# eggersn/DistributedFFT

Measured on AMD Instinct MI355X. Metric: 3D FFT GFLOP/s (5N^3 log2 N^3 per direction), forward+inverse, higher is better.
Workload: dtype f64

## Files before the change

### distributedfft_amd/__init__.py

```python
from ._lib import DfftError, LIB_PATH
from .api import (All2All, Comm, Configurations, DeviceBuffer, FORWARD, GlobalSize, INVERSE, MPI_Type, MPIcuFFT,
                  MPIcuFFT_Pencil, MPIcuFFT_Pencil_Opt1, MPIcuFFT_Slab, MPIcuFFT_Slab_Opt1, MPIcuFFT_Slab_Y_Then_ZX, MPIcuFFT_Slab_Z_Then_YX,
                  MPIcuFFT_Slab_Z_Then_YX_Opt1, Partition, Partition_Dimensions,
                  Peer2Peer, Pencil_Partition, SPECTRAL_OP, Slab_Partition, Streams, Sync, axis_plan_info, fft1d_batched, kernel_info, last_placement_info)
```

### distributedfft_amd/_lib.py

```python
import ctypes as C
import os

_HERE = os.path.dirname(os.path.abspath(__file__))
LIB_PATH = os.environ.get("DFFT_AMD_LIBRARY") or os.path.join(_HERE, "libdfft_amd.so")

ALLTOALLV_FN = C.CFUNCTYPE(C.c_int, C.c_void_p, C.c_void_p, C.POINTER(C.c_size_t), C.POINTER(C.c_size_t),
                           C.c_void_p, C.POINTER(C.c_size_t), C.POINTER(C.c_size_t), C.POINTER(C.c_int),
                           C.c_int, C.c_int, C.c_void_p)
SENDRECV_LIST_FN = C.CFUNCTYPE(C.c_int, C.c_void_p, C.c_int, C.POINTER(C.c_int), C.POINTER(C.c_void_p), C.POINTER(C.c_size_t),
                               C.c_int, C.POINTER(C.c_int), C.POINTER(C.c_void_p), C.POINTER(C.c_size_t), C.c_void_p)


class Config(C.Structure):
    _fields_ = [("cuda_aware", C.c_int), ("warmup_rounds", C.c_int), ("comm_method", C.c_int),
                ("send_method", C.c_int), ("comm_method2", C.c_int), ("send_method2", C.c_int)]


class PassDesc(C.Structure):
    _fields_ = [("na", C.c_uint32), ("LB", C.c_uint32), ("nb", C.c_uint32), ("LA", C.c_uint32), ("T2shift", C.c_uint32),
                ("load_kind", C.c_int32), ("store_kind", C.c_int32), ("swap", C.c_int32), ("shift", C.c_int32),
                ("KS_in", C.c_uint64), ("KS_out", C.c_uint64), ("AS_in", C.c_uint64), ("AS_out", C.c_uint64),
                ("IA", C.c_uint64), ("IB", C.c_uint64), ("SK", C.c_uint64), ("SB", C.c_uint64),
                ("a_fastest", C.c_int32), ("xcd_swizzle", C.c_int32),
                ("in_off", C.c_uint64), ("out_off", C.c_uint64),
# ... 67 lines not shown
    ("dfft_enable_phase_timing", _i, [_vp, _i]),
    ("dfft_fft1d_batched", _i, [_i, _sz, _sz, _vp, _vp, _i, _vp]),
    ("dfft_fft1d_batched_ex", _i, [_i, _sz, _sz, _vp, _vp, _i, _vp, _i, _i]),
    ("dfft_get_pass_choices", _i, [_vp, C.POINTER(_i), C.POINTER(_i), C.POINTER(_i)]),
    ("dfft_debug_get_pass", _i, [_vp, C.c_char_p, _i, C.POINTER(PassDesc)]),
    ("dfft_debug_get_chain", _i, [_vp, _i, _i, C.POINTER(ChainStep), _i, C.POINTER(_i)]),
    ("dfft_debug_trace_chain", _i, [_vp, _i, _i, C.POINTER(TraceOp), _i, C.POINTER(_i)]),
    ("dfft_debug_get_point_table", _i, [_vp, C.c_char_p, _i, _i, C.POINTER(C.c_uint64), C.POINTER(C.c_uint32),
                                        C.POINTER(C.c_uint32), _sz, _psz]),
    ("dfft_last_error", C.c_char_p, []),
    ("dfft_version", C.c_char_p, []),
    ("dfft_kernel_info", _i, [_i, _sz, C.POINTER(_i), C.POINTER(_i), C.POINTER(_i), C.POINTER(_i)]),
    ("dfft_axis_plan_info", _i, [_i, _sz, _i, C.POINTER(_sz)]),
    ("dfft_malloc", _i, [_sz, _sz, C.POINTER(_vp)]),
    ("dfft_free", _i, [_vp]),
    ("dfft_last_placement_info", _i, [C.c_char_p, _sz]),
    ("dfft_tune_variants", _i, [_vp, _vp, _vp, _vp, C.POINTER(C.c_float), _i, C.POINTER(_i)]),
    ("dfft_tune_placement", _i, [_vp, _vp, _i, C.POINTER(_vp), C.POINTER(_vp), C.POINTER(C.c_float), _i, C.POINTER(_i)]),
]

_lib = None


def lib():
    global _lib
    if _lib is None:
        if not os.path.exists(LIB_PATH):
            raise ImportError(
                f"{LIB_PATH} is missing: build it with `python -c 'import __graft_entry__ as g; g.build()'` "
                "or `make -C distributedfft_amd/csrc` (hipcc, gfx950).  There is no CPU fallback.")
# ... 17 lines not shown
```

### distributedfft_amd/api.py

```python
import ctypes as C
from dataclasses import dataclass

from . import _lib
from ._lib import Config, DfftError, check, lib

Peer2Peer, All2All = 0, 1
Sync, Streams, MPI_Type = 0, 1, 2
FORWARD, INVERSE = -1, 1
SPECTRAL_OP = 2


class GlobalSize:

    def __init__(self, Nx, Ny, Nz):
        self.Nx, self.Ny, self.Nz = int(Nx), int(Ny), int(Nz)
        self.Nz_out = self.Nz // 2 + 1


class Partition:

    def __init__(self, P1=1, P2=1):
        self.P1, self.P2 = int(P1), int(P2)


# ... 83 lines not shown
            lib().dfft_free(C.c_void_p(self.address))
        self.address = 0

    def __del__(self):
        try:
            self.free()
        except Exception:
            pass


def last_placement_info():
    import json
    buf = C.create_string_buffer(1024)
    check(lib().dfft_last_placement_info(buf, 1024))
    return json.loads(buf.value.decode())


class Comm:

    def __init__(self, handle, nranks, rank=None, keep=None):
        self._h, self.nranks, self.rank, self._keep = handle, nranks, rank, keep

    @classmethod
    def local(cls, nranks):
        h = C.c_void_p()
        check(lib().dfft_comm_create_local(nranks, C.byref(h)))
        return cls(h, nranks)

    @classmethod
    def rccl(cls, unique_id, nranks, rank):
# ... 365 lines not shown
```

### distributedfft_amd/csrc/alloc.hip

```cpp
#include <hip/hip_runtime.h>
#include <stdint.h>
#include <stdio.h>
#include <stdlib.h>

#include <algorithm>
#include <atomic>
#include <chrono>
#include <map>
#include <mutex>
#include <string>
#include <vector>

#include "alloc.hpp"
#include "host_common.hpp"

namespace dfft {

struct DevAlloc { size_t bytes, chunk; int device; };
static std::mutex g_alloc_mu;
static std::map<void *, DevAlloc> g_allocs;

static std::atomic<uintptr_t> g_next_va{0};
static hipError_t reserve_fresh(void **va, size_t total, size_t align)
{
// ... 24 lines not shown
        std::lock_guard<std::mutex> lk(g_alloc_mu);
        auto it = g_allocs.find(ptr);
        if (it != g_allocs.end()) { rec = it->second; g_allocs.erase(it); }
    }
    if (!rec.chunk) { HIP_TRY(hipFree(ptr)); return 0; }
    int cur = -1;
    (void)hipGetDevice(&cur);
    const bool hop = rec.device >= 0 && cur >= 0 && rec.device != cur;
    if (hop) HIP_TRY(hipSetDevice(rec.device));
    hipError_t e = hipDeviceSynchronize();
    for (size_t off = 0; off < rec.bytes && e == hipSuccess; off += rec.chunk) e = hipMemUnmap(static_cast<char *>(ptr) + off, rec.chunk);
    if (e == hipSuccess) e = hipMemAddressFree(ptr, rec.bytes);
    if (hop) (void)hipSetDevice(cur);
    if (e != hipSuccess) { set_error(std::string("dfft_free: ") + hipGetErrorString(e)); return (int)e; }
    return 0;
}
struct AllocTimes { double create = 0, map = 0, release = 0; };
static thread_local AllocTimes g_alloc_times;
static double seconds_since(std::chrono::steady_clock::time_point t0) { return std::chrono::duration<double>(std::chrono::steady_clock::now() - t0).count(); }

int dev_alloc(size_t bytes, size_t chunk_mib, void **out, int spread)
{
    *out = nullptr;
    g_alloc_times = AllocTimes();
    if (!bytes) return fail(ERR_ARG, "zero-sized allocation");
    if (!chunk_mib) {
        int dev0 = -1;
        (void)hipGetDevice(&dev0);
        HIP_TRY(hipMalloc(out, bytes));
        std::lock_guard<std::mutex> lk(g_alloc_mu);
// ... 276 lines not shown
```

### distributedfft_amd/csrc/alloc.hpp

```cpp
#pragma once
#include <stddef.h>

namespace dfft {
int dev_alloc(size_t bytes, size_t chunk_mib, void **out, int spread = 1);
int dev_alloc_default(size_t bytes, void **out);
int dev_free(void *ptr);
size_t default_chunk_mib();
int placement_info_json(char *buf, size_t capacity);
}
```

### distributedfft_amd/csrc/dfft.hip

```cpp
#include "../../include/dfft_c.h"
#include "comm.hpp"
#include "dfft_internal.hpp"
#include "fft_pass.hip.h"

#include <math.h>
#include <stdlib.h>
#include <string.h>
#include <algorithm>
#include <atomic>
#include <chrono>
#include <complex>
#include <functional>
#include <map>
#include <mutex>
#include <string>
#include <vector>

#include "alloc.hpp"
#include "host_common.hpp"
#include "plan.hpp"

namespace dfft {

static thread_local std::string g_error;
// ... 266 lines not shown
        PassArgs A = P;
        natural_side(A, false);
        layout(A, true, qout);
        PassArgs L3 = A;
        L3.lb = 0; L3.real_mode = 0; L3.swap = 0; L3.shift = 0;
        natural_side(L3, true);
        L3.out = nullptr;
        TRY(level(L3, 1, true));
        PassArgs L4 = A;
        L4.lb = 6; L4.lbL = (uint32_t)ax.N; L4.lbK = (uint32_t)NK; L4.lbtab = ax.chirp; L4.real_mode = real_mode;
        TRY(level(L4, 2, qout));
    }
    return 0;
}

static int launch(dfft_plan *p, const Launch &L, int form, int axis, bool conj, const char *in, char *out, hipStream_t stream)
{
    if (L.args.ntiles == 0) return 0;
    const Axis &ax = p->ax[axis];
    PassArgs A = L.args;
    A.in = in + L.in_off; A.out = out + L.out_off; A.tw = ax.tw; A.debug = p->opt.debug;
    if (conj) A.swap = 1;
    fill_tables(p, L, A);
    const int real_mode = form == FORM_REAL_Z1 || form == FORM_REAL_LINES ? 1 : form == FORM_REAL_Z2 ? 2 : 0;
    const size_t NK = real_mode ? ax.N / 2 + 1 : ax.N;
    if (real_mode && (form == FORM_REAL_LINES ? p->yreal_native : p->zreal_native)) {
        A.tw2 = p->tw_zr;
        const bool z = form != FORM_REAL_LINES;
        const int M = (int)((z ? p->Nz : p->Ny) / 2), variant = z ? p->opt.real_variant : 0;
        const int r = p->prec == DFFT_F64 ? launch_real_f64(M, real_mode, variant, A, stream) : launch_real_f32(M, real_mode, variant, A, stream);
        if (r != 0) return fail(r == -1 ? ERR_UNSUPPORTED : r, "real pass launch failed for length " + std::to_string(2 * M));
        return 0;
    }
    if (!ax.bluestein) {
        if (real_mode) return fail(ERR_UNSUPPORTED, "real pass without a packed or Bluestein plan");
        return launch_pass(p->prec, (int)ax.N, form == FORM_FWD ? p->vfwd[axis] : form == FORM_INV ? p->vinv[axis] : 0, A, stream);
// ... 87 lines not shown
    if (C < 2) return 1;
    return want < 0 ? (C >= 3 ? 2 : 1) : (want > 1 ? 2 : 1);
}

static hipEvent_t pipe_event(dfft_plan *p, size_t i)
{
    Pipeline &pl = p->pl;
    while (pl.ev.size() <= i) {
        hipEvent_t e = nullptr;
        if (hipEventCreateWithFlags(&e, hipEventDisableTiming) != hipSuccess) return nullptr;
        pl.ev.push_back(e);
    }
    return pl.ev[i];
}

static const Chain &chain_of(const dfft_plan *p, int direction, int dims)
{
    const Pipeline &pl = p->pl;
    if (direction == DFFT_SPECTRAL_OP) return pl.spec;
    const bool fwd = direction != DFFT_INVERSE;
    if (dims == 3 && one_rank_alternative(p) && !(fwd ? pl.one_fwd : pl.one_inv).steps.empty()) return fwd ? pl.one_fwd : pl.one_inv;
    return fwd ? pl.fwd[dims - 1] : pl.inv[dims - 1];
}

std::vector<Launch> *pass_launches(dfft_plan *p, int k)
{
    static const int alt[6] = {G_SZ, G_SY, G_SX, -1, -1, -1};
    const int g = p->pl.single && one_rank_alternative(p) ? alt[k] : k;
    return g < 0 ? nullptr : &p->pl.groups[g].L;
}

static bool graph_replay(const dfft_plan *p) { return p->opt.graph && p->nranks == 1 && !p->timing && (p->stream || !p->stream_user); }

static bool through_level_scratch(const dfft_plan *p, int form, int axis)
{
// ... 38 lines not shown
    int xchg(int step, int chunk, int s, int ) { ops.push_back(trace_exchange(st, step, chunk, s)); return 0; }
    int record(int s, int e) { ops.push_back(trace_sync(2, s, e)); return 0; }
    int wait(int e, int s) { ops.push_back(trace_sync(3, s, e)); return 0; }
    int begin(int, int) { return 0; }
    int end(int) { return 0; }
};

struct HipSink {
    dfft_plan *p;
    const std::vector<Step> &st;
    int direction;
    void *out;
    const void *in;
    std::vector<dfft_trace_op> *log;
    hipStream_t S[4];
    int open(const StreamUse &use)
    {
        Pipeline &pl = p->pl;
        if (use.compute2 && !pl.compute_stream2) HIP_TRY(hipStreamCreateWithFlags(&pl.compute_stream2, hipStreamNonBlocking));
        if (use.comm && !pl.comm_stream) HIP_TRY(hipStreamCreateWithFlags(&pl.comm_stream, hipStreamNonBlocking));
        if (use.comm2 && !pl.comm_stream2) HIP_TRY(hipStreamCreateWithFlags(&pl.comm_stream2, hipStreamNonBlocking));
        S[S_MAIN] = p->stream; S[S_COMPUTE2] = pl.compute_stream2; S[S_COMM] = pl.comm_stream; S[S_COMM2] = pl.comm_stream2;
        return 0;
    }
    char *buf(int b) const
    {
        return b == BUF_IN ? const_cast<char *>(static_cast<const char *>(in)) : b == BUF_OUT ? static_cast<char *>(out)
                                                                               : static_cast<char *>(p->work_d) + (size_t)b * p->domainsize;
    }
    int kernel(int step, int chunk, int k, int s)
    {
        const Step &t = st[(size_t)step];
        const Group &g = p->pl.groups[t.group];
        if (log) log->push_back(trace_launch(p, st, step, chunk, k, s));
        if (t.group == G_XX) return launch_spectral(p, g.L[(size_t)k], buf(t.src), buf(t.dst), S[s]);
        return launch(p, g.L[(size_t)k], t.form, g.axis, t.conj, buf(t.src), buf(t.dst), S[s]);
    }
    int xchg(int step, int chunk, int s, int ready)
    {
        const Step &t = st[(size_t)step];
        const Pipeline &pl = p->pl;
        const int dir = t.tables ? t.tables : direction;
        const std::vector<A2A> &T = dir == DFFT_INVERSE ? (t.xchg == 1 ? pl.i1 : pl.i2) : (t.xchg == 1 ? pl.f1 : pl.f2);
        if (log) log->push_back(trace_exchange(st, step, chunk, s));
        return exchange_tables(p, t.xchg, T[(size_t)chunk], true, buf(t.dst), buf(st[(size_t)step + 1].src), S[s], s == S_COMM2 ? 1 : 0, 0,
                               pl.ev[(size_t)ready]);
    }
    int record(int s, int e)
    {
        hipEvent_t ev = pipe_event(p, (size_t)e);
        if (!ev) return fail(1, "hipEventCreate failed");
// ... 62 lines not shown
                TRY(sk.xchg((int)s1 - 1, c, Sx, ready));
                if (t.phase >= 0) TRY(sk.end(Sx));
                TRY(record(Sx, xdone[c]));
            }
        }
        xprev = st[s1 - 1].xchg; xn = nchunk;
        if (s1 == st.size() && spread) TRY(join(Sc2, Sc));
    }
    return 0;
}

static int trace_slot(int direction) { return direction == DFFT_SPECTRAL_OP ? 2 : direction == DFFT_INVERSE ? 1 : 0; }

static int run_chain(dfft_plan *p, int direction, int dims, void *out, const void *in)
{
    const Chain &ch = chain_of(p, direction, dims);
    if (ch.steps.empty())
        return direction == DFFT_SPECTRAL_OP ? fail(ERR_STATE, "plan was initialised without option spectral_op")
                                             : fail(ERR_UNSUPPORTED, "the Y_Then_ZX sequence is forward only (as in the reference)");
    const StreamUse use = streams_of(p, ch);
    p->nspans = 0; p->last_dir = direction == DFFT_INVERSE ? DFFT_INVERSE : DFFT_FORWARD;
    std::vector<dfft_trace_op> *log = nullptr;
    if (p->opt.trace) { log = &p->trace_log[trace_slot(direction)]; log->clear(); }
    HipSink sk{p, ch.steps, direction, out, in, log, {}};
    TRY(sk.open(use));
    return schedule_chain(p, ch, use, sk);
}

void graphs_clear(dfft_plan *p)
{
    for (auto &g : p->graphs) if (g.exec) (void)hipGraphExecDestroy(g.exec);
    p->graphs.clear();
}
template <typename F> static int run_graphed(dfft_plan *p, int kind, const void *in, void *out, F &&enqueue)
{
    if (!graph_replay(p) || !p->stream) return enqueue();
    dfft_plan::GraphEntry *e = nullptr;
    for (auto &g : p->graphs) if (g.kind == kind && g.in == in && g.out == out) { e = &g; break; }
    if (e && e->exec) { HIP_TRY(hipGraphLaunch(e->exec, p->stream)); return 0; }
// ... 177 lines not shown
    if (k == "mirror_inverse") return &o.mirror;
    if (k == "point_tables") return &o.tables;
    if (k == "uniform_tables") return &o.uniform_tables;
    if (k == "shift") return &o.shift;
    if (k == "debug_skip") return &o.debug;
    if (k == "real_variant") return &o.real_variant;
    if (k == "single_order") return &o.single_order;
    if (k == "single_layout") return &o.single_layout;
    if (k == "single_pad") return &o.single_pad;
    if (k == "native_mixed") return &o.native_mixed;
    if (k == "graph") return &o.graph;
    if (k == "spectral_layout") return &o.spectral;
    if (k == "spectral_op") return &o.spectral_op;
    if (k == "compute_streams") return &o.compute_streams;
    if (k == "trace") return &o.trace;
    for (int i = 0; i < 6; i++) {
        if (k == std::string("variant_") + kPassNames[i]) return &o.variant[i];
        if (k == std::string("order_") + kPassNames[i]) return &o.order[i];
    }
    return nullptr;
}
int dfft_set_option(dfft_plan *p, const char *key, long value)
{
    if (!p || !key) return fail(ERR_ARG, "null plan or key");
    int *slot = option_slot(p->opt, key);
    if (!slot) return fail(ERR_ARG, std::string("unknown option ") + key);
    if (std::string(key).rfind("variant_", 0) == 0 && (value < -1 || value > 15)) return fail(ERR_ARG, "variant_* must be -1 (the plan's choice) or 0..15");
    *slot = (int)value;
    graphs_clear(p);
    return 0;
}
long dfft_get_option(dfft_plan *p, const char *key)
{
    if (!p || !key) return -1;
    int *slot = option_slot(p->opt, key);
    return slot ? *slot : -1;
}

int dfft_plan_destroy(dfft_plan *p)
{
    if (!p) return 0;
    graphs_clear(p);
    if (p->work_owned && p->work_d) (void)dev_free(p->work_d);
    relay_cache_free(p->relay);
    for (auto &a : p->ax) axis_free(a);
    for (void *t : {p->tw_zr, p->tables_d}) if (t) (void)hipFree(t);
    for (auto &t : p->spans) { if (t.a) (void)hipEventDestroy(t.a); if (t.b) (void)hipEventDestroy(t.b); }
    for (auto &e : p->pl.ev) if (e) (void)hipEventDestroy(e);
    if (p->pl.comm_stream) (void)hipStreamDestroy(p->pl.comm_stream);
    if (p->pl.comm_stream2) (void)hipStreamDestroy(p->pl.comm_stream2);
    if (p->pl.compute_stream2) (void)hipStreamDestroy(p->pl.compute_stream2);
    if (p->stream_owned && p->stream) (void)hipStreamDestroy(p->stream);
    delete p;
    return 0;
}

int dfft_init(dfft_plan *p, size_t Nx, size_t Ny, size_t Nz, int P1, int P2, int c2c, int allocate)
{
    if (!p) return fail(ERR_ARG, "null plan");
    p->initialized = false;
    graphs_clear(p);
    relay_cache_free(p->relay);
    p->relay = nullptr;
    if (!Nx || !Ny || !Nz) return fail(ERR_ARG, "GlobalSize not initialized!");
    if (P1 < 1 || P2 < 1 || P1 * P2 != p->nranks) return fail(ERR_ARG, "Invalid Input Partition!");
    const bool zyx_kind = p->kind == DFFT_SLAB_Z_THEN_YX || p->kind == DFFT_SLAB_Z_THEN_YX_OPT1;
    const bool yzx = p->kind == DFFT_SLAB_Y_THEN_ZX;
    if ((p->kind == DFFT_SLAB || p->kind == DFFT_SLAB_OPT1 || zyx_kind || yzx) && P2 != 1)
        return fail(ERR_ARG, "slab decomposition needs P2 == 1");
    const bool zyx = zyx_kind && P1 > 1;
    if (P1 > MAXSEG || P2 > MAXSEG) return fail(ERR_UNSUPPORTED, "more than 32 ranks per exchange group");
    if ((size_t)P1 > Nx || (!zyx && (size_t)P1 > Ny) || (size_t)P2 > Ny) return fail(ERR_ARG, "partition larger than the grid");
    {
        Axis az, ay, axx;
        const bool mixed = p->opt.native_mixed != 0;
        const int tl = p->opt.two_level;
        const bool zr_native = !yzx && !c2c && tl != 1 && Nz >= 4 && Nz <= 4096 && Nz % 2 == 0 && (is_pow2(Nz) || mixed) &&
                               (p->prec == DFFT_F64 ? real_supported_f64((int)(Nz / 2)) : real_supported_f32((int)(Nz / 2)));
// ... 95 lines not shown
            for (const Launch &L : g.L) {
                const Axis &a = p->ax[g.axis];
                if (a.two) lvb = std::max(lvb, two_level_bytes(L.args, p->TL, a.N, p->esz));
                if (a.longb) lvb = std::max(lvb, long_bytes(L.args, p->TL, a.M, p->esz));
            }
        p->worksize_d = (p->worksize_d + 255) & ~(size_t)255;
        p->lv_off = p->worksize_d;
        p->lv_bytes = (lvb + 255) & ~(size_t)255;
        p->worksize_d += p->lv_bytes;
    }
    {
        PassInfo vi;
        auto has64 = [&](const Axis &a, int role) { return !a.bluestein && pass_info_f64((int)a.N, role, &vi); };
        auto has32 = [&](const Axis &a, int role) { return !a.bluestein && pass_info_f32((int)a.N, role, &vi); };
        for (int k = 0; k < 3; k++) p->vfwd[k] = p->vinv[k] = ROLE_DEFAULT;
        if (p->prec == DFFT_F64) {
            const size_t zs_local = p->zs.empty() ? p->Nzc : p->zs[p->zyx ? (size_t)p->rank % p->zs.size() : (size_t)p->pj % p->zs.size()];
            if (has64(p->ax[2], ROLE_STRIDED_READ) && zs_local % (size_t)p->TL == 0) p->vinv[2] = ROLE_STRIDED_READ;
            if (p->vinv[2] == ROLE_STRIDED_READ && p->P1 == 1 && has64(p->ax[2], ROLE_STRIDED_READ_FUSED)) p->vinv[2] = ROLE_STRIDED_READ_FUSED;
            const int zrole = has64(p->ax[0], ROLE_LINES) ? ROLE_LINES : has64(p->ax[0], ROLE_STREAM) ? ROLE_STREAM : ROLE_DEFAULT;
            if (p->c2c) p->vfwd[0] = p->vinv[0] = zrole;
            if (has64(p->ax[1], ROLE_STREAM)) p->vinv[1] = ROLE_STREAM;
            if (p->opt.spectral) {
                const int xrole = has64(p->ax[2], ROLE_LINES) ? ROLE_LINES : has64(p->ax[2], ROLE_STREAM) ? ROLE_STREAM : ROLE_DEFAULT;
                p->vfwd[2] = p->vinv[2] = xrole;
            }
        } else {
            if (p->c2c && has32(p->ax[0], ROLE_NATURAL_LOAD)) p->vfwd[0] = ROLE_NATURAL_LOAD;
            if (p->c2c && has32(p->ax[0], ROLE_NATURAL_STORE)) p->vinv[0] = ROLE_NATURAL_STORE;
            for (int ax = 1; ax <= 2; ax++)
                if (has32(p->ax[ax], ROLE_TILED)) p->vfwd[ax] = p->vinv[ax] = ROLE_TILED;
            if (has32(p->ax[1], ROLE_TRANSPOSED_STORE)) p->vinv[1] = ROLE_TRANSPOSED_STORE;
            if (p->nranks > 1 && p->ax[1].N >= 2048 && has32(p->ax[1], ROLE_TILED_STREAM)) p->vfwd[1] = ROLE_TILED_STREAM;
            if (p->nranks > 1 && p->ax[2].N >= 2048 && has32(p->ax[2], ROLE_TILED_STREAM)) p->vinv[2] = ROLE_TILED_STREAM;
            if (p->opt.spectral) {
                if (has32(p->ax[2], ROLE_NATURAL_STORE)) p->vfwd[2] = ROLE_NATURAL_STORE;
                if (has32(p->ax[2], ROLE_NATURAL_LOAD_TILED_STORE)) p->vinv[2] = ROLE_NATURAL_LOAD_TILED_STORE;
            }
        }
    }
// ... 88 lines not shown
    }
    for (const Chain *ch : {&chain_of(p, DFFT_FORWARD, 3), &chain_of(p, DFFT_INVERSE, 3), &chain_of(p, DFFT_SPECTRAL_OP, 3)}) {
        HipSink sk{p, ch->steps, DFFT_FORWARD, nullptr, nullptr, nullptr, {}};
        TRY(sk.open(streams_of(p, *ch)));
    }
    return 0;
}

int dfft_set_work_area(dfft_plan *p, void *device, void *host)
{
    (void)host;
    if (!p) return fail(ERR_ARG, "null plan");
    if (!p->initialized) return fail(ERR_STATE, "cannot set work area: plan not initialised");
    graphs_clear(p);
    if (p->work_owned && p->work_d) { (void)dev_free(p->work_d); p->work_d = nullptr; p->work_owned = false; }
    TRY(ensure_device_state(p));
    if (device) {
        p->work_d = device;
    } else {
        TRY(dev_alloc_default(p->worksize_d, &p->work_d));
        p->work_owned = true;
    }
    return 0;
}

int dfft_set_pipeline_chunks(dfft_plan *p, int chunks)
{
    if (!p) return fail(ERR_ARG, "null plan");
    if (chunks < 0) return fail(ERR_ARG, "chunks must be >= 0");
    p->opt.chunks = chunks;
    return 0;
}
int dfft_get_pipeline_chunks(const dfft_plan *p) { return p ? p->pl.C : 0; }

int dfft_set_stream(dfft_plan *p, void *hip_stream)
{
    if (!p) return fail(ERR_ARG, "null plan");
// ... 195 lines not shown
    const Launch *L = find_launch(p, name, index);
    if (!L) return fail(ERR_ARG, "the plan has no such launch");
    const PassArgs &A = L->args;
    memset(d, 0, sizeof(*d));
    d->na = A.na; d->LB = A.LB; d->nb = A.nb; d->LA = A.LA; d->T2shift = A.T2shift;
    d->load_kind = A.load_kind; d->store_kind = A.store_kind; d->swap = A.swap; d->shift = A.shift;
    d->KS_in = A.KS_in; d->KS_out = A.KS_out; d->AS_in = A.AS_in; d->AS_out = A.AS_out;
    d->IA = A.IA; d->IB = A.IB; d->SK = A.SK; d->SB = A.SB; d->a_fastest = A.a_fastest; d->xcd_swizzle = A.xcd_swizzle;
    d->in_off = L->in_off; d->out_off = L->out_off;
    d->lnseg = L->lseg.nseg; d->snseg = L->sseg.nseg;
    for (int s = 0; s < L->lseg.nseg; s++) { d->lstart[s] = L->lseg.start[s]; d->llen[s] = L->lseg.len[s]; d->lbase[s] = L->lseg.base[s]; }
    for (int s = 0; s < L->sseg.nseg; s++) { d->sstart[s] = L->sseg.start[s]; d->slen[s] = L->sseg.len[s]; d->sbase[s] = L->sseg.base[s]; }
    return 0;
}

int dfft_debug_get_chain(const dfft_plan *p, int direction, int dims, dfft_chain_step *steps, int capacity, int *count)
{
    if (!p || !p->initialized) return fail(ERR_STATE, "plan not initialised");
    const bool spec = direction == DFFT_SPECTRAL_OP && dims == 3;
    if (dims < 1 || dims > 3 || (direction != DFFT_FORWARD && direction != DFFT_INVERSE && !spec)) return fail(ERR_ARG, "bad direction or dims");
    const Chain &ch = chain_of(p, direction, dims);
    const std::vector<Step> &st = ch.steps;
    if (count) *count = (int)st.size();
    for (size_t i = 0; i < st.size() && (int)i < capacity; i++) {
        const Step &s = st[i];
        const Group &g = p->pl.groups[s.group];
        dfft_chain_step &d = steps[i];
        memset(&d, 0, sizeof(d));
        strncpy(d.group, g.name, sizeof(d.group) - 1);
        d.axis = g.axis; d.launches = (int32_t)g.L.size(); d.per_chunk = s.per_chunk;
        d.src = s.src; d.dst = s.dst; d.conj = s.conj; d.form = s.form; d.exchange = s.xchg; d.split = ch.split;
        d.tables = s.tables ? s.tables : (direction == DFFT_INVERSE ? DFFT_INVERSE : DFFT_FORWARD);
    }
    return 0;
}

int dfft_debug_trace_chain(const dfft_plan *p, int direction, int dims, dfft_trace_op *ops, int capacity, int *count)
{
    if (!p || !p->initialized) return fail(ERR_STATE, "plan not initialised");
    const bool spec = direction == DFFT_SPECTRAL_OP && (dims == 3 || dims == 0);
    if (dims < 0 || dims > 3 || (direction != DFFT_FORWARD && direction != DFFT_INVERSE && !spec)) return fail(ERR_ARG, "bad direction or dims");
    std::vector<dfft_trace_op> dry;
    if (dims > 0) {
        const Chain &ch = chain_of(p, direction, dims);
        DrySink sk{p, ch.steps, dry};
        TRY(schedule_chain(p, ch, streams_of(p, ch), sk));
    }
    const std::vector<dfft_trace_op> &v = dims > 0 ? dry : p->trace_log[trace_slot(direction)];
    if (count) *count = (int)v.size();
    for (size_t i = 0; i < v.size() && (int)i < capacity; i++) ops[i] = v[i];
    return 0;
}

int dfft_get_pass_choices(const dfft_plan *p, int variant[6], int order[6], int addr64[6])
{
    if (!p || !p->initialized) return fail(ERR_STATE, "plan not initialised");
    for (int k = 0; k < 6; k++) {
        const std::vector<Launch> *v = pass_launches(const_cast<dfft_plan *>(p), k);
        const Launch *L = v && !v->empty() ? &(*v)[0] : nullptr;
// ... 142 lines not shown
    for (int k = 0; k < 8; k++) info[k] = 0;
    info[0] = a.longb ? 3 : a.two ? 2 : a.bluestein ? 1 : 0;
    info[1] = a.M;
    if (a.longb) a = Axis(a.lv[0]);
    for (size_t k = 0; k < a.lv.size(); k++) { info[2 + 3 * k] = a.lv[k].N; info[3 + 3 * k] = a.lv[k].M; info[4 + 3 * k] = a.lv[k].bluestein; }
    return 0;
}

int dfft_malloc(size_t bytes, size_t chunk_mib, void **ptr)
{
    if (!ptr) return fail(ERR_ARG, "null pointer");
    if (chunk_mib == DFFT_CHUNK_DEFAULT) return dev_alloc_default(bytes, ptr);
    return dev_alloc(bytes, chunk_mib, ptr);
}
int dfft_free(void *ptr) { return dev_free(ptr); }
int dfft_last_placement_info(char *buf, size_t capacity)
{
    if (!buf || !capacity) return fail(ERR_ARG, "null buffer");
    return placement_info_json(buf, capacity);
}

}
```

### distributedfft_amd/csrc/pipeline.hip

```cpp
#include <string.h>

#include <algorithm>

#include "host_common.hpp"
#include "plan.hpp"

using namespace dfft;

static PassArgs pass_args(int TL, size_t na, size_t LB, int load_kind, int store_kind, int swap)
{
    PassArgs A;
    memset(&A, 0, sizeof(A));
    A.na = (uint32_t)na; A.LB = (uint32_t)LB; A.nb = (uint32_t)((LB + TL - 1) / TL); A.ntiles = A.na * A.nb;
    A.load_kind = load_kind; A.store_kind = store_kind; A.swap = swap; A.T2shift = ilog2(TL);
    return A;
}

static void set_shift(const dfft_plan *p, PassArgs &X)
{
    const uint32_t TL = (uint32_t)p->TL;
    if (p->opt.shift == 0) return;
    if (p->ax[2].bluestein) return;
    if (p->prec != DFFT_F64 && p->opt.shift != 2) return;
    if (X.AS_out % TL == 0 || X.KS_out % TL != 0 || X.LB < TL) return;
    X.shift = 1;
    X.nb += 1;
    X.ntiles = X.na * X.nb;
}

static std::vector<Launch> &group(Pipeline &pl, int g, size_t n)
{
    pl.groups[g].L.assign(n, Launch());
    return pl.groups[g].L;
}

static void clear(Pipeline &pl)
{
    for (auto &g : pl.groups) g.L.clear();
    for (Chain *c : {&pl.fwd[0], &pl.fwd[1], &pl.fwd[2], &pl.inv[0], &pl.inv[1], &pl.inv[2], &pl.one_fwd, &pl.one_inv, &pl.spec}) *c = Chain();
    pl.single = false;
}

static void seg_push(SegTable &t, size_t start, size_t len, size_t base_elems)
{
    int s = t.nseg++;
    t.start[s] = (uint32_t)start;
    t.len[s] = (uint32_t)len;
    t.base[s] = base_elems;
}

int build_pipeline(dfft_plan *p, Pipeline &pl)
{
    const int TL = p->TL, P1 = p->P1, P2 = p->P2, C = pl.C;
    const size_t xs = p->xs[p->pi], ys = p->ys[p->pj], zs = p->zs[p->pj], yo = p->yo[p->pi];
// ... 183 lines not shown
        const int isrc = P1 > 1 ? (P2 > 1 ? 1 : E) : xd, idst = P2 > 1 ? E : (P1 > 1 ? 1 : 0), zsrc = P2 > 1 ? (P1 > 1 ? 0 : 1) : idst;
        pl.spec.steps = {{G_FZ, zf, BUF_IN, E, -1, x1, false, 1, false, DFFT_FORWARD},
                         {G_FY, FORM_FWD, ysrc, ydst, -1, x2, false, 1, false, DFFT_FORWARD},
                         {G_XX, FORM_FIXED, xsrc, xd, -1, x2, true, 1, false, DFFT_INVERSE},
                         {G_IY, FORM_INV, isrc, idst, -1, x1, true, 1, false, DFFT_INVERSE},
                         {G_IZ, zi, zsrc, BUF_OUT, -1, 0, P2 == 1, 1, false, DFFT_INVERSE}};
        pl.spec.split = true;
    }
    pl.fwd[0].steps = {{G_PZ1, zf, BUF_IN, BUF_OUT}};
    pl.inv[0].steps = {{G_QZ1, zi, BUF_IN, BUF_OUT}};
    pl.fwd[1].steps = {{G_FZ, zf, BUF_IN, 0, -1, x1}, {G_PY2, FORM_FWD, x1, BUF_OUT, -1, 0, P2 == 1}};
    pl.inv[1].steps = {{G_QY2, FORM_INV, BUF_IN, 0, -1, x1}, {G_IZ, zi, x1, BUF_OUT, -1, 0, P2 == 1}};
    if (p->nranks == 1 && p->c2c)
        pl.one_inv.steps = {{G_FZ, FORM_FWD, BUF_IN, 0, 4, 0, false, 1, true}, {G_FY, FORM_FWD, 0, BUF_IN, 2, 0, true, 1, true},
                            {G_FX, FORM_FWD, BUF_IN, BUF_OUT, 0, 0, true, 1, true}};
    return 0;
}

int build_pipeline_zyx(dfft_plan *p, Pipeline &pl)
{
    const int TL = p->TL, P = p->P1, C = pl.C, r = p->pi;
    const size_t xs = p->xs[r], zs = p->zs[r];
    const size_t Ny = p->Ny, Nzc = p->Nzc, e = p->esz;
    const size_t zline_bytes = p->c2c ? p->Nz * e : p->Nz * (e / 2);
    auto base = [&](size_t na, size_t LB, int lk, int sk, int swap) { return pass_args(TL, na, LB, lk, sk, swap); };
    std::vector<size_t> xl, x0;
    split(xs, C, xl, x0);
    std::vector<std::vector<size_t>> xlq(P), x0q(P);
    for (int q = 0; q < P; q++) split(p->xs[q], C, xlq[q], x0q[q]);
    std::vector<std::vector<size_t>> blk(C, std::vector<size_t>(P, 0));
// ... 192 lines not shown
```

### distributedfft_amd/csrc/plan.hpp

```cpp
#pragma once
#include <hip/hip_runtime.h>
#include <stddef.h>
#include <stdint.h>

#include <string>
#include <vector>

#include "../../include/dfft_c.h"
#include "comm.hpp"
#include "dfft_internal.hpp"
#include "fft_pass.hip.h"

namespace dfft {

inline void split(size_t n, int p, std::vector<size_t> &size, std::vector<size_t> &start)
{
    size.assign(p, n / p);
    start.assign(p, 0);
    for (size_t i = 0; i < n % p; i++) size[i]++;
    size_t off = 0;
    for (int i = 0; i < p; i++) { start[i] = off; off += size[i]; }
}

inline bool is_pow2(size_t n) { return n && !(n & (n - 1)); }
// ... 61 lines not shown
    bool whole = false;
    int per_chunk = 1;
    bool conj = false;
    int tables = 0;
};
struct Chain {
    std::vector<Step> steps;
    bool split = false;
};

struct Pipeline {
    int C = 1;
    Group groups[NGROUPS] = {{"fz", 0}, {"fy", 1}, {"fx", 2}, {"ix", 2}, {"iy", 1}, {"iz", 0}, {"pz1", 0}, {"qz1", 0}, {"py2", 1},
                             {"qy2", 1}, {"zy", 1}, {"ziy", 1}, {"zix", 2}, {"yz", 0}, {"sz", 0}, {"sx", 2}, {"sy", 1}, {"xx", 2}};
    Chain fwd[3], inv[3], one_fwd, one_inv;
    Chain spec;
    bool single = false;
    size_t single_work_elems = 0;
    std::vector<A2A> f1, f2, i2, i1;
    std::vector<hipEvent_t> ev;
    hipStream_t comm_stream = nullptr;
    hipStream_t comm_stream2 = nullptr;
    hipStream_t compute_stream2 = nullptr;
};

struct TimedSpan { hipEvent_t a = nullptr, b = nullptr; int phase = 0; bool used = false; };

struct Options {
    int chunks = 0;
    int mirror = 0;
    int tables = 1;
    int uniform_tables = 1;
    int shift = -1;
    int debug = 0;
    int real_variant = 0;
    int single_order = -1;
    int single_layout = 1;
    int single_pad = 128;
    int graph = 0;
    int native_mixed = 1;
    int two_level = 0;
    int spectral = 0;
    int spectral_op = 0;
    int compute_streams = -1;
    int trace = 0;
    int order[6] = {-1, -1, -1, -1, -1, -1};
    int variant[6] = {-1, -1, -1, -1, -1, -1};
};

struct dfft_plan {
    int kind = DFFT_PENCIL_OPT1, prec = DFFT_F64;
    dfft_config cfg{};
    dfft_comm *comm = nullptr;
    int rank = 0, nranks = 1;
    bool initialized = false, c2c = false;
    bool spectral_mirror = false;
    bool zyx = false;
    bool yzx = false;
    size_t Nyc = 0;
    size_t Nx = 0, Ny = 0, Nz = 0, Nzc = 0;
    int P1 = 1, P2 = 1, pi = 0, pj = 0;
    int TL = 8;
    std::vector<size_t> xs, xstart, ys, ystart, zs, zstart, yo, yostart;
    size_t esz = 16, domain_elems = 0, domainsize = 0, worksize_d = 0;
    void *work_d = nullptr;
    bool work_owned = false;
    dfft::Axis ax[3];
    bool zreal_native = false;
    bool yreal_native = false;
    size_t lv_off = 0, lv_bytes = 0;
    void *tw_zr = nullptr;
    void *tables_d = nullptr;
    hipStream_t stream = nullptr;
    bool stream_owned = false;
    bool stream_user = false;
    std::vector<size_t> sc1, sd1, rc1, rd1, sc2, sd2, rc2, rd2;
    std::vector<int> group1, group2;
    dfft::RelayCache *relay = nullptr;
    int vfwd[3] = {0, 0, 0}, vinv[3] = {0, 0, 0};
    Options opt;
    Pipeline pl;
    bool timing = false;
    std::vector<TimedSpan> spans;
    size_t nspans = 0;
    int last_dir = -1;
    std::vector<dfft_trace_op> trace_log[3];
    dfft_spectral_op op{};
    struct GraphEntry { int kind; const void *in; void *out; int uses; hipGraphExec_t exec; };
    std::vector<GraphEntry> graphs;
};

int build_pipeline(dfft_plan *p, Pipeline &pl);
int build_pipeline_zyx(dfft_plan *p, Pipeline &pl);
int build_pipeline_yzx(dfft_plan *p, Pipeline &pl);
int build_pipeline_single(dfft_plan *p, Pipeline &pl);
int check_ready(dfft_plan *p);
inline bool one_rank_alternative(const dfft_plan *p) { return p->nranks == 1 && p->c2c && !p->opt.mirror && !p->spectral_mirror; }
std::vector<Launch> *pass_launches(dfft_plan *p, int k);
void graphs_clear(dfft_plan *p);
```

### distributedfft_amd/csrc/tune.hip

```cpp
#include <stdlib.h>
#include <string.h>

#include <algorithm>
#include <functional>
#include <string>
#include <vector>

#include "alloc.hpp"
#include "host_common.hpp"
#include "plan.hpp"

using namespace dfft;

extern "C" {

static int placement_measure(dfft_plan *p, const void *in, void *out, void *back, int reps, float *ms)
{
    auto once = [&](float *sum) -> int {
        float ph[5];
        if (p->c2c) TRY(dfft_exec_c2c(p, out, const_cast<void *>(in), DFFT_FORWARD)); else TRY(dfft_exec_r2c(p, out, in));
        int n = dfft_get_phase_times(p, ph, 5);
        float acc = 0;
        for (int i = 0; i < n; i += 2) acc += ph[i];
        if (back) {
// ... 29 lines not shown
    }
    return 0;
}

static int tune_variants(dfft_plan *p, const void *in, void *o, void *b, float &best, const std::function<void(float)> &note)
{
    if (p->zyx || p->yzx) return 0;
    const bool shared = one_rank_alternative(p);
    auto launches = [&](int k, const std::function<void(Launch &)> &f) {
        if (std::vector<Launch> *v = pass_launches(p, k)) for (Launch &L : *v) f(L);
    };
    auto axis_of = [](int k) { return k < 3 ? k : 5 - k; };
    auto slot = [&](int k) -> int & { return k < 3 ? p->vfwd[k] : p->vinv[5 - k]; };
    auto usable = [&](int k) { return !(k >= 3 && (!b || shared)); };
    float t[6], total = 0;
    auto cost = [&](const float *tt, int k) { return shared && b ? tt[k] + tt[5 - k] : tt[k]; };

    {
        int keep[6];
        float tb[6] = {0, 0, 0, 0, 0, 0}, td[4][6];
        for (int k = 0; k < 6; k++) {
            keep[k] = -1;
            launches(k, [&](Launch &L) { if (keep[k] < 0) keep[k] = (L.args.a_fastest ? 1 : 0) + (L.args.xcd_swizzle ? 2 : 0); });
        }
        auto apply = [&](int k, int d) { launches(k, [&](Launch &L) { L.args.a_fastest = d & 1; L.args.xcd_swizzle = (d >> 1) & 1; }); };
        auto tunable = [&](int k) { return keep[k] >= 0 && p->opt.order[k] < 0 && usable(k); };
        for (int d = 0; d < 4; d++) {
            for (int k = 0; k < 6; k++) if (tunable(k)) apply(k, d);
            TRY(tune_trial(p, in, o, b, td[d], &total));
            note(total);
// ... 154 lines not shown
```

### include/dfft_c.h

```cpp
#ifndef DFFT_C_H
#define DFFT_C_H

#include <stddef.h>
#include <stdint.h>

#ifdef __cplusplus
extern "C" {
#endif

typedef struct dfft_plan dfft_plan;
typedef struct dfft_comm dfft_comm;

enum dfft_kind {
    DFFT_SLAB = 0,
    DFFT_SLAB_OPT1 = 1,
    DFFT_PENCIL = 2,
    DFFT_PENCIL_OPT1 = 3,
    DFFT_SLAB_Z_THEN_YX = 4,
    DFFT_SLAB_Z_THEN_YX_OPT1 = 5,
    DFFT_SLAB_Y_THEN_ZX = 6
};
enum dfft_precision { DFFT_F32 = 0, DFFT_F64 = 1 };
enum dfft_direction { DFFT_FORWARD = -1, DFFT_INVERSE = 1 };
#define DFFT_SPECTRAL_OP 2
// ... 128 lines not shown
    int32_t scratch;
} dfft_trace_op;
int dfft_debug_trace_chain(const dfft_plan *plan, int direction, int dims, dfft_trace_op *ops, int capacity, int *count);
int dfft_debug_get_point_table(const dfft_plan *plan, const char *name, int index, int store, uint64_t *base,
                               uint32_t *ln, uint32_t *aux, size_t capacity, size_t *count);

const char *dfft_last_error(void);
const char *dfft_version(void);
int dfft_kernel_info(int precision, size_t N, int *threads, int *lds_bytes, int *points_per_thread,
                     int *lines_per_workgroup);
int dfft_axis_plan_info(int precision, size_t N, int two_level, size_t info[8]);

#define DFFT_CHUNK_DEFAULT ((size_t)-1)
int dfft_malloc(size_t bytes, size_t chunk_mib, void **ptr);
int dfft_free(void *ptr);
int dfft_last_placement_info(char *buf, size_t capacity);
int dfft_tune_placement(dfft_plan *plan, const void *in, int tries, void **out, void **back, float *report_ms,
                        int max_report, int *n_report);
int dfft_tune_variants(dfft_plan *plan, const void *in, void *out, void *back, float *report_ms, int max_report, int *n_report);

#ifdef __cplusplus
}
#endif
#endif
```

Measured before the change: 9575.

## Route single-rank intermediates through a private slice and pick variants by buffer placement

```diff
diff --git a/distributedfft_amd/__init__.py b/distributedfft_amd/__init__.py
--- a/distributedfft_amd/__init__.py
+++ b/distributedfft_amd/__init__.py
@@ -2,4 +2,4 @@
 from .api import (All2All, Comm, Configurations, DeviceBuffer, FORWARD, GlobalSize, INVERSE, MPI_Type, MPIcuFFT,
                   MPIcuFFT_Pencil, MPIcuFFT_Pencil_Opt1, MPIcuFFT_Slab, MPIcuFFT_Slab_Opt1, MPIcuFFT_Slab_Y_Then_ZX, MPIcuFFT_Slab_Z_Then_YX,
                   MPIcuFFT_Slab_Z_Then_YX_Opt1, Partition, Partition_Dimensions,
-                  Peer2Peer, Pencil_Partition, SPECTRAL_OP, Slab_Partition, Streams, Sync, axis_plan_info, fft1d_batched, kernel_info, last_placement_info)
+                  Peer2Peer, Pencil_Partition, SPECTRAL_OP, Slab_Partition, Streams, Sync, axis_plan_info, fft1d_batched, kernel_info, last_placement_info, owns)
diff --git a/distributedfft_amd/_lib.py b/distributedfft_amd/_lib.py
--- a/distributedfft_amd/_lib.py
+++ b/distributedfft_amd/_lib.py
@@ -105,6 +105,7 @@
     ("dfft_axis_plan_info", _i, [_i, _sz, _i, C.POINTER(_sz)]),
     ("dfft_malloc", _i, [_sz, _sz, C.POINTER(_vp)]),
     ("dfft_free", _i, [_vp]),
+    ("dfft_owns", _i, [_vp]),
     ("dfft_last_placement_info", _i, [C.c_char_p, _sz]),
     ("dfft_tune_variants", _i, [_vp, _vp, _vp, _vp, C.POINTER(C.c_float), _i, C.POINTER(_i)]),
     ("dfft_tune_placement", _i, [_vp, _vp, _i, C.POINTER(_vp), C.POINTER(_vp), C.POINTER(C.c_float), _i, C.POINTER(_i)]),
diff --git a/distributedfft_amd/api.py b/distributedfft_amd/api.py
--- a/distributedfft_amd/api.py
+++ b/distributedfft_amd/api.py
@@ -121,6 +121,10 @@
     buf = C.create_string_buffer(1024)
     check(lib().dfft_last_placement_info(buf, 1024))
     return json.loads(buf.value.decode())
+
+
+def owns(x):
+    return bool(lib().dfft_owns(_ptr(x)))
 
 
 class Comm:
diff --git a/distributedfft_amd/csrc/alloc.hip b/distributedfft_amd/csrc/alloc.hip
--- a/distributedfft_amd/csrc/alloc.hip
+++ b/distributedfft_amd/csrc/alloc.hip
@@ -62,6 +62,14 @@
     if (hop) (void)hipSetDevice(cur);
     if (e != hipSuccess) { set_error(std::string("dfft_free: ") + hipGetErrorString(e)); return (int)e; }
     return 0;
+}
+bool dev_owns(const void *ptr)
+{
+    std::lock_guard<std::mutex> lk(g_alloc_mu);
+    auto it = g_allocs.upper_bound(const_cast<void *>(ptr));
+    if (it == g_allocs.begin()) return false;
+    --it;
+    return it->second.chunk != 0 && static_cast<const char *>(ptr) < static_cast<const char *>(it->first) + it->second.bytes;
 }
 struct AllocTimes { double create = 0, map = 0, release = 0; };
 static thread_local AllocTimes g_alloc_times;
diff --git a/distributedfft_amd/csrc/alloc.hpp b/distributedfft_amd/csrc/alloc.hpp
--- a/distributedfft_amd/csrc/alloc.hpp
+++ b/distributedfft_amd/csrc/alloc.hpp
@@ -5,6 +5,7 @@
 int dev_alloc(size_t bytes, size_t chunk_mib, void **out, int spread = 1);
 int dev_alloc_default(size_t bytes, void **out);
 int dev_free(void *ptr);
+bool dev_owns(const void *ptr);
 size_t default_chunk_mib();
 int placement_info_json(char *buf, size_t capacity);
 }
diff --git a/distributedfft_amd/csrc/dfft.hip b/distributedfft_amd/csrc/dfft.hip
--- a/distributedfft_amd/csrc/dfft.hip
+++ b/distributedfft_amd/csrc/dfft.hip
@@ -304,12 +304,13 @@
     return 0;
 }
 
-static int launch(dfft_plan *p, const Launch &L, int form, int axis, bool conj, const char *in, char *out, hipStream_t stream)
+static int launch(dfft_plan *p, const Launch &L, int form, int axis, bool conj, const char *in, char *out, hipStream_t stream, int a_fastest = -1)
 {
     if (L.args.ntiles == 0) return 0;
     const Axis &ax = p->ax[axis];
     PassArgs A = L.args;
     A.in = in + L.in_off; A.out = out + L.out_off; A.tw = ax.tw; A.debug = p->opt.debug;
+    if (a_fastest >= 0) A.a_fastest = a_fastest;
     if (conj) A.swap = 1;
     fill_tables(p, L, A);
     const int real_mode = form == FORM_REAL_Z1 || form == FORM_REAL_LINES ? 1 : form == FORM_REAL_Z2 ? 2 : 0;
@@ -427,11 +428,45 @@
     return pl.ev[i];
 }
 
-static const Chain &chain_of(const dfft_plan *p, int direction, int dims)
+static bool private_eligible(const dfft_plan *p)
+{
+    return p->opt.private_intermediates != 0 && one_rank_alternative(p) && !p->pl.single && !p->pl.priv_fwd.steps.empty() && !p->priv_refused &&
+           !p->opt.refuse_private_slice && (p->work_owned || !p->work_d);
+}
+static bool wants_private(const dfft_plan *p, int direction, const void *out, const void *in)
+{
+    if (!private_eligible(p)) return false;
+    return p->opt.private_intermediates == 1 || !dev_owns(direction == DFFT_INVERSE ? in : out);
+}
+static bool ensure_private_slice(dfft_plan *p)
+{
+    if (p->priv_d) return true;
+    size_t free_b = 0, total_b = 0;
+    if (hipMemGetInfo(&free_b, &total_b) != hipSuccess || p->domainsize > free_b / 2 || dev_alloc_default(p->domainsize, &p->priv_d) != 0) {
+        (void)hipGetLastError();
+        p->priv_d = nullptr;
+        p->priv_refused = true;
+        return false;
+    }
+    return true;
+}
+int fz_rule_a_fastest(const dfft_plan *p, const void *out, const void *in)
+{
+    return dev_owns(wants_private(p, DFFT_FORWARD, out, in) && p->priv_d ? p->priv_d : out) ? 1 : 0;
+}
+static void private_slice_free(dfft_plan *p)
+{
+    if (p->priv_d) (void)dev_free(p->priv_d);
+    p->priv_d = nullptr;
+    p->priv_refused = false;
+}
+
+static const Chain &chain_of(const dfft_plan *p, int direction, int dims, bool priv = false)
 {
     const Pipeline &pl = p->pl;
     if (direction == DFFT_SPECTRAL_OP) return pl.spec;
     const bool fwd = direction != DFFT_INVERSE;
+    if (dims == 3 && priv) return fwd ? pl.priv_fwd : pl.priv_inv;
     if (dims == 3 && one_rank_alternative(p) && !(fwd ? pl.one_fwd : pl.one_inv).steps.empty()) return fwd ? pl.one_fwd : pl.one_inv;
     return fwd ? pl.fwd[dims - 1] : pl.inv[dims - 1];
 }
@@ -500,6 +535,7 @@
     const void *in;
     std::vector<dfft_trace_op> *log;
     hipStream_t S[4];
+    char *w1 = nullptr;
     int open(const StreamUse &use)
     {
         Pipeline &pl = p->pl;
@@ -512,7 +548,7 @@
     char *buf(int b) const
     {
         return b == BUF_IN ? const_cast<char *>(static_cast<const char *>(in)) : b == BUF_OUT ? static_cast<char *>(out)
-                                                                               : static_cast<char *>(p->work_d) + (size_t)b * p->domainsize;
+               : b == 1 && w1 ? w1 : static_cast<char *>(p->work_d) + (size_t)b * p->domainsize;
     }
     int kernel(int step, int chunk, int k, int s)
     {
@@ -520,7 +556,8 @@
         const Group &g = p->pl.groups[t.group];
         if (log) log->push_back(trace_launch(p, st, step, chunk, k, s));
         if (t.group == G_XX) return launch_spectral(p, g.L[(size_t)k], buf(t.src), buf(t.dst), S[s]);
-        return launch(p, g.L[(size_t)k], t.form, g.axis, t.conj, buf(t.src), buf(t.dst), S[s]);
+        const int a_fastest = p->fz_by_dst && t.group == G_FZ ? (dev_owns(buf(t.dst)) ? 1 : 0) : -1;
+        return launch(p, g.L[(size_t)k], t.form, g.axis, t.conj, buf(t.src), buf(t.dst), S[s], a_fastest);
     }
     int xchg(int step, int chunk, int s, int ready)
     {
@@ -613,7 +650,8 @@
 
 static int run_chain(dfft_plan *p, int direction, int dims, void *out, const void *in)
 {
-    const Chain &ch = chain_of(p, direction, dims);
+    const bool priv = dims == 3 && direction != DFFT_SPECTRAL_OP && wants_private(p, direction, out, in) && ensure_private_slice(p);
+    const Chain &ch = chain_of(p, direction, dims, priv);
     if (ch.steps.empty())
         return direction == DFFT_SPECTRAL_OP ? fail(ERR_STATE, "plan was initialised without option spectral_op")
                                              : fail(ERR_UNSUPPORTED, "the Y_Then_ZX sequence is forward only (as in the reference)");
@@ -622,6 +660,7 @@
     std::vector<dfft_trace_op> *log = nullptr;
     if (p->opt.trace) { log = &p->trace_log[trace_slot(direction)]; log->clear(); }
     HipSink sk{p, ch.steps, direction, out, in, log, {}};
+    if (priv) sk.w1 = static_cast<char *>(p->priv_d);
     TRY(sk.open(use));
     return schedule_chain(p, ch, use, sk);
 }
@@ -829,6 +868,8 @@
     if (k == "spectral_op") return &o.spectral_op;
     if (k == "compute_streams") return &o.compute_streams;
     if (k == "trace") return &o.trace;
+    if (k == "private_intermediates") return &o.private_intermediates;
+    if (k == "refuse_private_slice") return &o.refuse_private_slice;
     for (int i = 0; i < 6; i++) {
         if (k == std::string("variant_") + kPassNames[i]) return &o.variant[i];
         if (k == std::string("order_") + kPassNames[i]) return &o.order[i];
@@ -857,6 +898,7 @@
     if (!p) return 0;
     graphs_clear(p);
     if (p->work_owned && p->work_d) (void)dev_free(p->work_d);
+    private_slice_free(p);
     relay_cache_free(p->relay);
     for (auto &a : p->ax) axis_free(a);
     for (void *t : {p->tw_zr, p->tables_d}) if (t) (void)hipFree(t);
@@ -877,6 +919,7 @@
     graphs_clear(p);
     relay_cache_free(p->relay);
     p->relay = nullptr;
+    private_slice_free(p);
     if (!Nx || !Ny || !Nz) return fail(ERR_ARG, "GlobalSize not initialized!");
     if (P1 < 1 || P2 < 1 || P1 * P2 != p->nranks) return fail(ERR_ARG, "Invalid Input Partition!");
     const bool zyx_kind = p->kind == DFFT_SLAB_Z_THEN_YX || p->kind == DFFT_SLAB_Z_THEN_YX_OPT1;
@@ -1002,6 +1045,7 @@
         auto has64 = [&](const Axis &a, int role) { return !a.bluestein && pass_info_f64((int)a.N, role, &vi); };
         auto has32 = [&](const Axis &a, int role) { return !a.bluestein && pass_info_f32((int)a.N, role, &vi); };
         for (int k = 0; k < 3; k++) p->vfwd[k] = p->vinv[k] = ROLE_DEFAULT;
+        p->fy_by_work = p->fz_by_dst = false;
         if (p->prec == DFFT_F64) {
             const size_t zs_local = p->zs.empty() ? p->Nzc : p->zs[p->zyx ? (size_t)p->rank % p->zs.size() : (size_t)p->pj % p->zs.size()];
             if (has64(p->ax[2], ROLE_STRIDED_READ) && zs_local % (size_t)p->TL == 0) p->vinv[2] = ROLE_STRIDED_READ;
@@ -1012,6 +1056,12 @@
             if (p->opt.spectral) {
                 const int xrole = has64(p->ax[2], ROLE_LINES) ? ROLE_LINES : has64(p->ax[2], ROLE_STREAM) ? ROLE_STREAM : ROLE_DEFAULT;
                 p->vfwd[2] = p->vinv[2] = xrole;
+            }
+            if (p->nranks == 1 && p->c2c && !p->pl.single && !p->opt.spectral && p->pl.C == 1) {
+                if (p->ax[2].N == 1024 && has64(p->ax[2], ROLE_STREAM)) p->vfwd[2] = ROLE_STREAM;
+                p->fy_by_work = p->ax[1].N == 1024 && has64(p->ax[1], ROLE_STREAM) && p->opt.variant[1] < 0;
+                p->fz_by_dst = p->ax[0].N == 1024 && !p->ax[0].bluestein && p->opt.order[0] < 0;
+                if (p->fz_by_dst) for (Launch &L : p->pl.groups[G_FZ].L) L.args.a_fastest = 1;
             }
         } else {
             if (p->c2c && has32(p->ax[0], ROLE_NATURAL_LOAD)) p->vfwd[0] = ROLE_NATURAL_LOAD;
@@ -1130,6 +1180,7 @@
     if (!p->initialized) return fail(ERR_STATE, "cannot set work area: plan not initialised");
     graphs_clear(p);
     if (p->work_owned && p->work_d) { (void)dev_free(p->work_d); p->work_d = nullptr; p->work_owned = false; }
+    private_slice_free(p);
     TRY(ensure_device_state(p));
     if (device) {
         p->work_d = device;
@@ -1137,6 +1188,7 @@
         TRY(dev_alloc_default(p->worksize_d, &p->work_d));
         p->work_owned = true;
     }
+    if (p->fy_by_work) p->vfwd[1] = dev_owns(p->work_d) ? ROLE_STREAM : ROLE_DEFAULT;
     return 0;
 }
 
@@ -1362,12 +1414,17 @@
     return 0;
 }
 
+static bool debug_private(const dfft_plan *p, int direction, int dims)
+{
+    return dims == 3 && direction != DFFT_SPECTRAL_OP && p->opt.private_intermediates == 1 && private_eligible(p);
+}
+
 int dfft_debug_get_chain(const dfft_plan *p, int direction, int dims, dfft_chain_step *steps, int capacity, int *count)
 {
     if (!p || !p->initialized) return fail(ERR_STATE, "plan not initialised");
     const bool spec = direction == DFFT_SPECTRAL_OP && dims == 3;
     if (dims < 1 || dims > 3 || (direction != DFFT_FORWARD && direction != DFFT_INVERSE && !spec)) return fail(ERR_ARG, "bad direction or dims");
-    const Chain &ch = chain_of(p, direction, dims);
+    const Chain &ch = chain_of(p, direction, dims, debug_private(p, direction, dims));
     const std::vector<Step> &st = ch.steps;
     if (count) *count = (int)st.size();
     for (size_t i = 0; i < st.size() && (int)i < capacity; i++) {
@@ -1390,7 +1447,7 @@
     if (dims < 0 || dims > 3 || (direction != DFFT_FORWARD && direction != DFFT_INVERSE && !spec)) return fail(ERR_ARG, "bad direction or dims");
     std::vector<dfft_trace_op> dry;
     if (dims > 0) {
-        const Chain &ch = chain_of(p, direction, dims);
+        const Chain &ch = chain_of(p, direction, dims, debug_private(p, direction, dims));
         DrySink sk{p, ch.steps, dry};
         TRY(schedule_chain(p, ch, streams_of(p, ch), sk));
     }
@@ -1563,6 +1620,7 @@
     return dev_alloc(bytes, chunk_mib, ptr);
 }
 int dfft_free(void *ptr) { return dev_free(ptr); }
+int dfft_owns(const void *ptr) { return dev_owns(ptr) ? 1 : 0; }
 int dfft_last_placement_info(char *buf, size_t capacity)
 {
     if (!buf || !capacity) return fail(ERR_ARG, "null buffer");
diff --git a/distributedfft_amd/csrc/pipeline.hip b/distributedfft_amd/csrc/pipeline.hip
--- a/distributedfft_amd/csrc/pipeline.hip
+++ b/distributedfft_amd/csrc/pipeline.hip
@@ -37,7 +37,7 @@
 static void clear(Pipeline &pl)
 {
     for (auto &g : pl.groups) g.L.clear();
-    for (Chain *c : {&pl.fwd[0], &pl.fwd[1], &pl.fwd[2], &pl.inv[0], &pl.inv[1], &pl.inv[2], &pl.one_fwd, &pl.one_inv, &pl.spec}) *c = Chain();
+    for (Chain *c : {&pl.fwd[0], &pl.fwd[1], &pl.fwd[2], &pl.inv[0], &pl.inv[1], &pl.inv[2], &pl.one_fwd, &pl.one_inv, &pl.priv_fwd, &pl.priv_inv, &pl.spec}) *c = Chain();
     pl.single = false;
 }
 
@@ -251,6 +251,12 @@
     if (p->nranks == 1 && p->c2c)
         pl.one_inv.steps = {{G_FZ, FORM_FWD, BUF_IN, 0, 4, 0, false, 1, true}, {G_FY, FORM_FWD, 0, BUF_IN, 2, 0, true, 1, true},
                             {G_FX, FORM_FWD, BUF_IN, BUF_OUT, 0, 0, true, 1, true}};
+    if (p->nranks == 1 && p->c2c) {
+        pl.priv_fwd.steps = {{G_FZ, FORM_FWD, BUF_IN, 1, 0, 0}, {G_FY, FORM_FWD, 1, 0, 2, 0}, {G_FX, FORM_FWD, 0, BUF_OUT, 4, 0, true}};
+        pl.priv_fwd.split = true;
+        pl.priv_inv.steps = {{G_FZ, FORM_FWD, BUF_IN, 0, 4, 0, false, 1, true}, {G_FY, FORM_FWD, 0, 1, 2, 0, true, 1, true},
+                             {G_FX, FORM_FWD, 1, BUF_OUT, 0, 0, true, 1, true}};
+    }
     return 0;
 }
 
diff --git a/distributedfft_amd/csrc/plan.hpp b/distributedfft_amd/csrc/plan.hpp
--- a/distributedfft_amd/csrc/plan.hpp
+++ b/distributedfft_amd/csrc/plan.hpp
@@ -99,6 +99,7 @@
     Group groups[NGROUPS] = {{"fz", 0}, {"fy", 1}, {"fx", 2}, {"ix", 2}, {"iy", 1}, {"iz", 0}, {"pz1", 0}, {"qz1", 0}, {"py2", 1},
                              {"qy2", 1}, {"zy", 1}, {"ziy", 1}, {"zix", 2}, {"yz", 0}, {"sz", 0}, {"sx", 2}, {"sy", 1}, {"xx", 2}};
     Chain fwd[3], inv[3], one_fwd, one_inv;
+    Chain priv_fwd, priv_inv;
     Chain spec;
     bool single = false;
     size_t single_work_elems = 0;
@@ -128,6 +129,8 @@
     int spectral = 0;
     int spectral_op = 0;
     int compute_streams = -1;
+    int private_intermediates = -1;
+    int refuse_private_slice = 0;
     int trace = 0;
     int order[6] = {-1, -1, -1, -1, -1, -1};
     int variant[6] = {-1, -1, -1, -1, -1, -1};
@@ -150,6 +153,8 @@
     size_t esz = 16, domain_elems = 0, domainsize = 0, worksize_d = 0;
     void *work_d = nullptr;
     bool work_owned = false;
+    void *priv_d = nullptr;
+    bool priv_refused = false;
     dfft::Axis ax[3];
     bool zreal_native = false;
     bool yreal_native = false;
@@ -163,6 +168,7 @@
     std::vector<int> group1, group2;
     dfft::RelayCache *relay = nullptr;
     int vfwd[3] = {0, 0, 0}, vinv[3] = {0, 0, 0};
+    bool fy_by_work = false, fz_by_dst = false;
     Options opt;
     Pipeline pl;
     bool timing = false;
@@ -182,4 +188,5 @@
 int check_ready(dfft_plan *p);
 inline bool one_rank_alternative(const dfft_plan *p) { return p->nranks == 1 && p->c2c && !p->opt.mirror && !p->spectral_mirror; }
 std::vector<Launch> *pass_launches(dfft_plan *p, int k);
+int fz_rule_a_fastest(const dfft_plan *p, const void *out, const void *in);
 void graphs_clear(dfft_plan *p);
diff --git a/distributedfft_amd/csrc/tune.hip b/distributedfft_amd/csrc/tune.hip
--- a/distributedfft_amd/csrc/tune.hip
+++ b/distributedfft_amd/csrc/tune.hip
@@ -67,6 +67,11 @@
     auto slot = [&](int k) -> int & { return k < 3 ? p->vfwd[k] : p->vinv[5 - k]; };
     auto usable = [&](int k) { return !(k >= 3 && (!b || shared)); };
     float t[6], total = 0;
+    if (p->fz_by_dst) {
+        const int a = fz_rule_a_fastest(p, o, in);
+        launches(0, [&](Launch &L) { L.args.a_fastest = a; });
+        p->fz_by_dst = false;
+    }
     auto cost = [&](const float *tt, int k) { return shared && b ? tt[k] + tt[5 - k] : tt[k]; };
 
     {
diff --git a/include/dfft_c.h b/include/dfft_c.h
--- a/include/dfft_c.h
+++ b/include/dfft_c.h
@@ -166,6 +166,7 @@
 #define DFFT_CHUNK_DEFAULT ((size_t)-1)
 int dfft_malloc(size_t bytes, size_t chunk_mib, void **ptr);
 int dfft_free(void *ptr);
+int dfft_owns(const void *ptr);
 int dfft_last_placement_info(char *buf, size_t capacity);
 int dfft_tune_placement(dfft_plan *plan, const void *in, int tries, void **out, void **back, float *report_ms,
                         int max_report, int *n_report);
```

Result: no change. 9594 (median of 4 runs) (+0.2%).
